# awslabs/dgl-ke

Measured on NVIDIA H100. Metric: edges/sec TransE_l2 d=400 neg=200 at 1/2/4/8 H100 vs ref CPU; HBM GB/s %peak, higher is better.
Workload: dtype f32

## Files before the change

### dgl-ke_b200/csrc/kge_abi.cu

```cuda
#include <cstdio>
#include <unistd.h>
#include <cstdarg>
#include <cstring>
#include <cstdlib>
#include <map>
#include <mutex>
#include <new>
#include <utility>
#include <cuda.h>
#include "kge_common.cuh"

namespace kge {

namespace {
thread_local char g_err[512] = "";
}

int fail(int code, const char* fmt, ...) {
  va_list ap;
  va_start(ap, fmt);
  vsnprintf(g_err, sizeof(g_err), fmt, ap);
  va_end(ap);
  return code;
}
// ... 182 lines not shown
  if (cfg->batch <= 0 || cfg->chunk_size <= 0 || cfg->neg_sample_size <= 0)
    return fail(KGE_ERR_INVALID_ARG, "batch/chunk_size/neg_sample_size must be positive");
  if (cfg->batch % cfg->chunk_size != 0)
    return fail(KGE_ERR_INVALID_ARG, "batch %lld is not a multiple of chunk_size %d", (long long)cfg->batch, cfg->chunk_size);
  const int D = cfg->entity_dim, Dr = cfg->relation_dim;
  if (D <= 0 || Dr <= 0) return fail(KGE_ERR_INVALID_ARG, "dims must be positive");
  if (D % 4 != 0 || Dr % 4 != 0)
    return fail(KGE_ERR_UNSUPPORTED, "row lengths must be multiples of 4 floats (16-byte vector/TMA access): D_e=%d D_r=%d", D, Dr);
  switch (cfg->model) {
    case KGE_TRANSE_L1: case KGE_TRANSE_L2: case KGE_DISTMULT:
      if (Dr != D) return fail(KGE_ERR_INVALID_ARG, "model needs relation_dim == entity_dim (%d vs %d)", Dr, D);
      break;
    case KGE_COMPLEX:
      if (Dr != D || D % 8 != 0) return fail(KGE_ERR_INVALID_ARG, "ComplEx needs relation_dim == entity_dim, a multiple of 8");
      break;
    case KGE_ROTATE:
      if (D != 2 * Dr || D % 8 != 0) return fail(KGE_ERR_INVALID_ARG, "RotatE needs entity_dim == 2*relation_dim (-de), a multiple of 8");
      break;
    case KGE_RESCAL:
      if (Dr != D * D) return fail(KGE_ERR_INVALID_ARG, "RESCAL needs relation_dim == entity_dim^2");
      if (D > 512) return fail(KGE_ERR_UNSUPPORTED, "RESCAL entity_dim %d > 512 is not implemented", D);
      break;
  }
  p->model = cfg->model; p->D = D; p->Dr = Dr;
  p->gamma = cfg->gamma; p->emb_init = cfg->emb_init; p->lr = cfg->lr;
  p->reg_coef = cfg->reg_coef; p->reg_norm = cfg->reg_norm;
  p->adversarial = cfg->adversarial; p->adv_temperature = cfg->adv_temperature;
  p->neg_head = cfg->neg_head ? 1 : 0;
  p->B = cfg->batch; p->Cs = cfg->chunk_size; p->Ns = cfg->neg_sample_size;
  p->C = (int)(cfg->batch / cfg->chunk_size);
  p->neg_deg = cfg->neg_deg_sample ? 1 : 0;
  if (p->neg_deg) p->Ns += p->Cs;
  p->Nn = (long long)p->C * p->Ns;
  p->U = n_nodes >= 0 ? n_nodes : 2 * p->B;
  p->U_dev = nullptr;
  p->rel_deferred = 0; p->rel_dense = 0; p->use_nc = 1; p->fused = 0; p->nc_staged = 0;
  if (cfg->loss_genre < KGE_LOSS_LOGSIGMOID || cfg->loss_genre > KGE_LOSS_BCE)
    return fail(KGE_ERR_INVALID_ARG, "loss_genre %d is not a kge_loss_t", cfg->loss_genre);
  if (cfg->pairwise && cfg->loss_genre != KGE_LOSS_HINGE && cfg->loss_genre != KGE_LOSS_LOGISTIC)
    return fail(KGE_ERR_INVALID_ARG, "pairwise needs the Hinge or the Logistic criterion (loss.py:61-62)");
  if (cfg->pairwise && cfg->adversarial)
    return fail(KGE_ERR_INVALID_ARG, "loss cannot be pairwise and adversarial sampled (base_loss.py:83-84)");
  p->hinge = cfg->loss_genre == KGE_LOSS_HINGE ? 1 : 0;
  p->margin = cfg->margin;
  p->pairwise = cfg->pairwise ? 1 : 0;
  return KGE_OK;
}

size_t align_up(size_t x, size_t a = 256) { return (x + a - 1) / a * a; }

struct CarveOpt {
  bool force_tiles = false;
  bool want_scores = true;
};

bool use_fused(kge_context* h, const StepParams& p) {
  return h->engine != 0 && h->fused_mode != 0 && fused_supported(p);
}

bool use_umma(kge_context* h, const StepParams& p) {
  return h->engine != 0 && umma_supported(p);
}

int carve(kge_context* h, const StepParams& p, StepWs* w, cudaStream_t stream, const CarveOpt& opt = CarveOpt()) {
  const size_t BD = (size_t)p.B * p.D, ND = (size_t)p.Nn * p.D, BNs = (size_t)p.B * p.Ns;
  const size_t B = (size_t)p.B, Nn = (size_t)p.Nn, U = (size_t)(p.U > 0 ? p.U : 0);
  const bool um = !opt.force_tiles && use_umma(h, p);
  const bool fused = p.fused != 0;
  const FusedHilo hl = fused ? fused_hilo(p) : FusedHilo{false, false};
  const size_t sA = B * slab_blocks(p.D) * 32 + 8192, sB = Nn * slab_blocks(p.D) * 32 + 8192;
  const size_t sV = B * slab_blocks(p.Ns) * 32 + 8192;
  const size_t sAT = (size_t)p.C * slab_blocks(p.Cs) * p.D * 32 + 8192, sBT = (size_t)p.C * slab_blocks(p.Ns) * p.D * 32 + 8192;
  const size_t sVT = (size_t)p.C * slab_blocks(p.Cs) * p.Ns * 32 + 8192;
  struct Slot { float** ptr; size_t floats; bool on; };
  const Slot slots[] = {
      {&w->NG, (U ? 2 * B : 0) * p.D, true},
      {&w->A, BD, !(um || fused)}, {&w->Bn, ND, true}, {&w->GA, BD, true}, {&w->GR, B * p.Dr, !p.rel_dense},
      {&w->S, BNs, !fused || opt.want_scores}, {&w->V, BNs, !fused},
      {&w->pos, B, true}, {&w->gpos, B, true}, {&w->pnorm, B, true}, {&w->a2, B, true}, {&w->b2, Nn, true},
      {&w->rowsum, B, true}, {&w->colsum, Nn, true}, {&w->pl, B, true}, {&w->nl, B, true}, {&w->wbar, 4, true},
      {&w->gsr, B, true}, {&w->gsn, Nn, true}, {&w->colpart, (size_t)ceil_div(p.Cs, 128) * Nn, fused},
      {&w->Mt, BD, p.model == KGE_RESCAL},
      {&w->Ahi, sA, um && (!fused || hl.a)}, {&w->Alo, sA, um && (!fused || hl.a)}, {&w->Af, sA, fused && !hl.a},
      {&w->Bhi, sB, um}, {&w->Blo, sB, um},
      {&w->Vhi, sV, um && !fused}, {&w->Vlo, sV, um && !fused},
      {&w->AhiT, sAT, um}, {&w->AloT, sAT, um}, {&w->BhiT, sBT, um}, {&w->BloT, sBT, um},
      {&w->VhiT, sVT, um && (!fused || hl.v)}, {&w->VloT, sVT, um && (!fused || hl.v)}, {&w->VT, sVT, fused},
      {&w->NC, U * p.D, p.use_nc != 0},
      {&w->regp, B + Nn + (U ? 2 * B : 0), true},
  };
  size_t need = 0;
  for (const Slot& s : slots)
    if (s.on) need += align_up(s.floats * sizeof(float));
  if (need > h->arena.bytes) {
    if (int rc = h->arena.resize(need + need / 4, stream, "step workspace")) return rc;
    h->ng_ptr = nullptr; h->ng_floats = 0;
  }
  size_t off = 0;
  for (const Slot& s : slots) {
    *s.ptr = s.on ? (float*)(h->arena.as<char>() + off) : nullptr;
    if (s.on) off += align_up(s.floats * sizeof(float));
  }
  w->red_partial = h->red_partial; w->red_ticket = (unsigned int*)(h->red_partial + 192);
  w->sync_ctr = (unsigned int*)(h->red_partial + 200);
  w->rg = nullptr; w->rgs = nullptr;
  return KGE_OK;
}

int ensure_rel_dense(kge_context* h, const TableView& rel, StepWs* w, cudaStream_t stream) {
  const size_t bytes = ((size_t)rel.num_rows * rel.dim + (size_t)rel.num_rows) * sizeof(float);
  if (bytes != h->rel_dense.bytes) {
    if (int rc = h->rel_dense.resize(bytes, stream, "relation gradient sums")) return rc;
    KGE_CUDA_OK(cudaMemsetAsync(h->rel_dense.p, 0, bytes, stream));
  }
  w->rg = h->rel_dense.as<float>();
  w->rgs = w->rg + (size_t)rel.num_rows * rel.dim;
  return KGE_OK;
}

LaunchCtx lctx(kge_context* h, void* stream) { return LaunchCtx{(cudaStream_t)stream, &h->launches, h->num_sms, &h->prof}; }

void ensure_ng_zero(kge_context* h, const StepParams& p, const StepWs& w, const LaunchCtx& c, bool force) {
  size_t n = (size_t)2 * p.B * p.D;
  if (force || h->ng_dirty || h->ng_ptr != w.NG || h->ng_floats < n) {
    launch_fill_zero(c, w.NG, (long long)n);
    h->ng_ptr = w.NG;
    h->ng_dirty = false;
  }
  h->ng_floats = n;
}

int check_batch(const kge_batch_t* b, const StepParams& p) {
  if (!b) return fail(KGE_ERR_INVALID_ARG, "batch is null");
  if (!b->node_ids || !b->head_local || !b->tail_local || !b->rel_ids || !b->neg_ids)
    return fail(KGE_ERR_INVALID_ARG, "batch has null index arrays");
  if (b->n_nodes < 0 && b->n_nodes_dev) return KGE_OK;
  if (b->n_nodes <= 0 || b->n_nodes > 2 * p.B) return fail(KGE_ERR_INVALID_ARG, "n_nodes=%lld out of (0, 2*batch]", (long long)b->n_nodes);
  return KGE_OK;
}
// ... 231 lines not shown
  if (rc) return rc;
  p.model = KGE_DISTMULT;
  DeviceGuard g(h->device);
  StepWs w{};
  rc = carve(h, p, &w, (cudaStream_t)stream);
  if (rc) return rc;
  h->ng_ptr = nullptr;
  w.V = dneg;
  w.gpos = dpos;
  launch_loss(lctx(h, stream), p, pos, neg, wt, w, log4, false);
  KGE_CUDA_OK(cudaGetLastError());
  h->have_last = false;
  return KGE_OK;
}

KGE_API int kge_adagrad(kge_handle_t h, const kge_table_t* table, const int64_t* idx, const float* grad, int64_t n, float lr,
                void* stream) {
  if (!h) return fail(KGE_ERR_INVALID_ARG, "handle is null");
  if (n < 0) return fail(KGE_ERR_INVALID_ARG, "n < 0");
  if (n == 0) return KGE_OK;
  if (!idx || !grad) return fail(KGE_ERR_INVALID_ARG, "null pointer");
  TableView v;
  int rc = make_view(table, &v, "adagrad");
  if (rc) return rc;
  DeviceGuard g(h->device);
  launch_adagrad(lctx(h, stream), v, (const long long*)idx, grad, n, lr);
  KGE_CUDA_OK(cudaGetLastError());
  return KGE_OK;
}

static int forward_backward_impl(kge_handle_t h, const kge_step_cfg_t* cfg, const kge_table_t* ent, const kge_table_t* rel,
                                 const kge_batch_t* batch, float* log4, void* stream, bool fused_step) {
  if (!h) return fail(KGE_ERR_INVALID_ARG, "handle is null");
  StepParams p;
  int rc = make_params(cfg, batch ? batch->n_nodes : 0, &p);
  if (rc) return rc;
  rc = check_batch(batch, p);
  if (rc) return rc;
  if (batch->n_nodes < 0) p.U_dev = (const long long*)batch->n_nodes_dev;
  p.rel_deferred = h->rel_deferred;
  TableView ve, vr;
  if ((rc = make_view(ent, &ve, "entity"))) return rc;
  if ((rc = make_view(rel, &vr, "relation"))) return rc;
  if (ve.dim != p.D || vr.dim != p.Dr)
    return fail(KGE_ERR_INVALID_ARG, "table dims (%d,%d) do not match cfg (%d,%d)", ve.dim, vr.dim, p.D, p.Dr);
  DeviceGuard g(h->device);
  p.fused = use_fused(h, p) ? 1 : 0;
  p.use_nc = (fused_step && ve.n_shards == 1) ? 0 : 1;
  p.rel_dense = (fused_step && p.model != KGE_RESCAL &&
                 (p.rel_deferred ? (h->ext_rg != nullptr) : ((size_t)vr.num_rows * (size_t)vr.dim <= ((size_t)64 << 20)))) ? 1 : 0;
  StepWs w{};
  CarveOpt opt;
  opt.want_scores = !fused_step;
  if ((rc = carve(h, p, &w, (cudaStream_t)stream, opt))) return rc;
  if (p.rel_dense && p.rel_deferred) { w.rg = h->ext_rg; w.rgs = h->ext_rgs; }
  else if (p.rel_dense && (rc = ensure_rel_dense(h, vr, &w, (cudaStream_t)stream))) return rc;
  LaunchCtx c = lctx(h, stream);
  BatchView b = bview(batch);
  if (p.neg_deg) {
    if (ve.n_shards != 1) return fail(KGE_ERR_UNSUPPORTED, "--neg_deg_sample needs a single-shard entity table");
    const size_t bytes = (size_t)p.Nn * sizeof(long long);
    if (bytes > h->negdeg_ids.bytes && (rc = h->negdeg_ids.resize(bytes, (cudaStream_t)stream, "neg_deg_sample id list")))
      return rc;
    launch_negdeg_ids(c, p, b, b.neg_ids, h->negdeg_ids.as<long long>());
    b.neg_ids = h->negdeg_ids.as<long long>();
  }
  ensure_ng_zero(h, p, w, c, false);
  const bool stageable = fused_step && p.fused && p.use_nc;
  float* const arena_nc = w.NC;
  h->pf.take_staged(*batch, stageable, p, w);
  const FusedPrefetch* pfp = nullptr;
  if ((rc = h->pf.arm_next(stageable, p, w, arena_nc, (cudaStream_t)stream, &pfp))) return rc;
  if (p.use_nc && !p.nc_staged) launch_gather_nodes(c, p, ve, b, w);
  if ((rc = (p.model == KGE_RESCAL) ? launch_rescal_prep(c, p, ve, vr, b, w) : launch_prep(c, p, ve, vr, b, w))) return rc;
  if (p.neg_deg) launch_negdeg_zero_reg(c, p, w);
  float* logdst = log4 ? log4 : h->dev_log4;
  if (p.fused) {
    launch_wbar(c, p, b.edge_weight, w);
    if ((rc = fused_launch(c, p, w, 0, b.edge_weight, fused_step ? nullptr : w.S, h->dump_v, &ve, b.neg_ids, pfp))) return rc;
    if ((rc = fused_launch(c, p, w, 1, b.edge_weight, nullptr,
                           h->dump_v ? h->dump_v + (size_t)p.B * p.Ns : nullptr, &ve, b.neg_ids, pfp))) return rc;
  } else {
    if ((rc = run_score(h, c, p, w))) return rc;
    if (p.neg_deg) launch_negdeg_mask_scores(c, p, w);
    launch_wbar(c, p, b.edge_weight, w);
    launch_loss_rows(c, p, w.pos, w.S, b.edge_weight, w);
    if (p.neg_deg) launch_negdeg_mask_coef(c, p, w);
    launch_colsum(c, p, w);
    if (use_umma(h, p)) {
      if ((rc = umma_grad(c, p, w, false))) return rc;
      if ((rc = umma_grad(c, p, w, true))) return rc;
    } else {
      launch_grad_a(c, p, w);
      launch_grad_b(c, p, w);
    }
    if (p.neg_deg) launch_negdeg_scatter(c, p, ve, b, w);
  }
  if (p.model == KGE_RESCAL) launch_rescal_chain(c, p, ve, vr, b, w);
  else launch_chain(c, p, ve, vr, b, w);
  if (fused_step && p.rel_deferred && !p.rel_dense && h->ext_rg) launch_rel_grad_dense(c, p, b, w, h->ext_rg, h->ext_rgs);
  if (!fused_step) launch_reduce_log(c, p, b.edge_weight, w, logdst, true);
  KGE_CUDA_OK(cudaGetLastError());
  h->last_p = p; h->last_w = w; h->last_b = b; h->last_ent = ve; h->last_rel = vr; h->have_last = true;
  h->ng_dirty = true;
  return KGE_OK;
}
// ... 432 lines not shown
```

### dgl-ke_b200/csrc/kge_common.cuh

```cuda
#pragma once
#include <cuda_runtime.h>
#include <stdint.h>
#include "../../include/kge_b200.h"

namespace kge {

constexpr int kWarp = 32;

struct TableView {
  float* emb[KGE_MAX_SHARDS];
  float* state[KGE_MAX_SHARDS];
  long long rows_per_shard;
  long long num_rows;
  int n_shards;
  int dim;
};

__device__ __forceinline__ float* row_ptr(const TableView& t, long long id) {
  if (t.n_shards == 1) return t.emb[0] + id * (long long)t.dim;
  int s = (int)(id / t.rows_per_shard);
  return t.emb[s] + (id - (long long)s * t.rows_per_shard) * (long long)t.dim;
}
__device__ __forceinline__ float* state_ptr(const TableView& t, long long id) {
  if (t.n_shards == 1) return t.state[0] + id;
// ... 324 lines not shown
void launch_adagrad(const LaunchCtx&, const TableView& t, const long long* idx, const float* grad,
                    long long n, float lr);
void launch_node_grad_with_reg(const LaunchCtx&, const StepParams&, const TableView& ent,
                               const BatchView&, const StepWs&, float* out);
void launch_fill_zero(const LaunchCtx&, float* p, long long n);
void launch_rel_grad_dense(const LaunchCtx&, const StepParams&, const BatchView&, const StepWs&, float* rg, float* rgs);
void launch_rel_apply_dense(const LaunchCtx&, const TableView& rel, float* rg, float* rgs, float lr);

void launch_negdeg_ids(const LaunchCtx&, const StepParams&, const BatchView&, const long long* sampled, long long* out);
void launch_negdeg_zero_reg(const LaunchCtx&, const StepParams&, const StepWs&);
void launch_negdeg_mask_scores(const LaunchCtx&, const StepParams&, const StepWs&);
void launch_negdeg_mask_coef(const LaunchCtx&, const StepParams&, const StepWs&);
void launch_negdeg_scatter(const LaunchCtx&, const StepParams&, const TableView& ent, const BatchView&, const StepWs&);

struct RankParams {
  const float* S;
  long long ld, Q, N;
  const float* pos;
  long long base;
  const long long* cand;
  long long chunk;
  const long long* kept;
  const long long* rel;
  const long long* keys;
  const int* vals;
  long long n_keys, n_rel;
  long long* cnt;
};
void launch_rank_count(const LaunchCtx&, const RankParams&);
void launch_rank_finish(const LaunchCtx&, const long long* cnt, long long Q, long long* rank_out, double* acc);

int launch_rescal_prep(const LaunchCtx&, const StepParams&, const TableView& ent, const TableView& rel,
                       const BatchView&, const StepWs&);
void launch_rescal_prep_dense(const LaunchCtx&, const StepParams&, const float* head, const float* relr,
                              const float* tail, const StepWs&, bool want_pos, bool want_a);
void launch_rescal_chain(const LaunchCtx&, const StepParams&, const TableView& ent, const TableView& rel,
                         const BatchView&, const StepWs&);

bool umma_supported(const StepParams&);
int umma_score(const LaunchCtx&, const StepParams&, const StepWs&);
int umma_grad(const LaunchCtx&, const StepParams&, const StepWs&, bool side_b);

struct FusedPrefetch {
  const long long* node_ids;
  const long long* nU_dev;
  long long nU;
  const long long* neg_ids;
  long long nNeg;
  float* nc;
  float* bn;
};
bool fused_supported(const StepParams&);
int fused_prefetch_slots(const StepParams& p, int mode);
struct FusedHilo { bool a, v; };
FusedHilo fused_hilo(const StepParams& p);
int fused_launch(const LaunchCtx&, const StepParams&, const StepWs&, int mode, const float* wt, float* dumpS, float* dumpV,
                 const TableView* ent, const long long* neg_ids, const FusedPrefetch* pf);

}
```

### dgl-ke_b200/csrc/kge_fused.cu

```cuda
#include <cuda.h>
#include <cstdio>
#include <cstdlib>
#include <mutex>
#include "kge_common.cuh"
#include "kge_tc.cuh"

namespace kge {

using namespace tc;

namespace {

constexpr int kTileM = 128;
constexpr int kThreadsF = 384;
constexpr int kProducerWarp = 8;
constexpr int kHandoffWarp = 9;
constexpr int kMaxS1 = 4, kMaxS2 = 8;
constexpr int kMaxPf = 8;
constexpr uint32_t kRingBytes = 192 * 1024;
constexpr uint32_t kRingBytesP = 223 * 1024;
constexpr float kLog2e = 1.4426950408889634f;
constexpr float kLn2 = 0.6931471805599453f;

struct FusedArgs {
  int model, adversarial;
  float gamma, Tl2e, inv2B, uni;
  float reg_coef;
  int reg_norm;
  int C, Rx, Ry, D;
  int N1;
  int N2;
  int nblkD;
  int nS1, nS2;
  uint32_t stage1Bytes, stage2Bytes;
  float* VT;
  float *VhiT, *VloT;
  float* colpart;
  int ncolpart;
  const float* x2;
  const float* y2;
  const float* pos;
  const float* wt;
  const float* wbar;
  float *gpos, *rowsum, *pl, *nl;
  float* dumpS;
  float* dumpV;
  const float *Xhi, *Xlo;
  const long long* xids;
  TableView xtab;
  const float* xraw;
  float* gsn;
  float* out;
  int pf_slots;
  int pf_parity;
  int pf_lag;
  uint32_t pf_off, pf_row_bytes;
  const long long* pf_node_ids;
  const long long* pf_nU_dev;
  long long pf_nU, pf_nNeg;
  const long long* pf_neg_ids;
  float* pf_nc;
  float* pf_bn;
};

static __device__ __noinline__ float reg_grad_any(float b, int norm, float coef) { return reg_grad(b, norm, coef); }
__device__ __forceinline__ float reg_grad_fast(float b, int norm, float coef) {
  if (norm == 3) return 3.f * coef * fabsf(b) * b;
  return reg_grad_any(b, norm, coef);
}

__device__ __forceinline__ void epi_bar() { asm volatile("bar.sync 1, 256;" ::: "memory"); }

__device__ __forceinline__ void prefetch_rows(const FusedArgs& g, uint8_t* ring, uint64_t (*pf_full)[kMaxPf], int w, int lane) {
  const int S = g.pf_slots;
  const long long nU = g.pf_nU_dev ? *g.pf_nU_dev : g.pf_nU;
  const long long total = nU + g.pf_nNeg;
  const long long nhalf = total > g.pf_parity ? (total - g.pf_parity + 1) / 2 : 0;
  const long long stride = 2ll * gridDim.x, j0 = 2ll * blockIdx.x + w;
  const long long n = j0 < nhalf ? (nhalf - j0 + stride - 1) / stride : 0;
  uint8_t* slots = ring + g.pf_off + (size_t)w * S * g.pf_row_bytes;
  auto vrow = [&](long long k) { return g.pf_parity + 2 * (j0 + k * stride); };
  auto fetch_ids = [&](long long kb) {
    const long long k = kb + lane;
    if (k >= n) return 0ll;
    const long long v = vrow(k);
    return v < nU ? g.pf_node_ids[v] : g.pf_neg_ids[v - nU];
  };
// ... 401 lines not shown
        float acc2[NW / 2];
#pragma unroll
        for (int i = 0; i < NW / 2; ++i) acc2[i] = 0.f;
        uint32_t ah[2][4], al[2][4];
#pragma unroll 1
        for (int kb = 0; kb < nkb2; ++kb) {
          const uint32_t s = n2 % g.nS2;
          mbar_wait(&full2[s], (n2 / g.nS2) & 1);
          const uint32_t st = smem_u32(ring2 + (size_t)s * g.stage2Bytes);
          const uint64_t dYh = make_desc(st), dYl = make_desc(st + yBytes2);
          const int kleft = g.Ry - kb * 32;
          const int ksteps = kleft >= 32 ? 4 : (kleft >> 3);
#pragma unroll
          for (int ks = 0; ks < 4; ++ks) {
            const int j = kb * 4 + ks;
            if (ks < ksteps) {
              const uint64_t o = (uint64_t)(ks * 2);
              pos_kstep<NW>(acc2, ah[j & 1], al[j & 1], vw + j * 128, dYh + o, dYl + o);
              if (j > 0) {
                wgmma_wait<1>();
                reg_fence(ah[(j - 1) & 1]); reg_fence(al[(j - 1) & 1]);
                if (ks == 0 && lane == 0) mbar_arrive(&empty2[(n2 - 1) % g.nS2]);
              }
            }
          }
          ++n2;
        }
        wgmma_wait<0>();
        reg_fence(ah[0]); reg_fence(ah[1]); reg_fence(al[0]); reg_fence(al[1]);
        if (lane == 0) mbar_arrive(&empty2[(n2 - 1) % g.nS2]);
        reg_fence(acc2);
#pragma unroll
        for (int h = 0; h < 2; ++h) {
          const int m = m0 + rloc + 8 * h;
          if (m >= g.Rx) continue;
          float* orow = g.out + ((long long)c * g.Rx + m) * (long long)g.D;
#pragma unroll
          for (int j = 0; j < NW / 8; ++j) {
            const int k = d0 + 8 * j + 2 * q;
            if (k >= g.D) continue;
            *reinterpret_cast<float2*>(orow + k) = make_float2(acc2[4 * j + 2 * h] * rscal[h], acc2[4 * j + 2 * h + 1] * rscal[h]);
          }
        }
      }
      asm volatile("fence.proxy.async.shared::cta;" ::: "memory");
      __syncwarp();
      if (lane == 0) mbar_arrive(&vfree);
    }
  }
}

constexpr int kNegEpiLoads = 16;

template <int NW, bool FLAT>
__global__ void __launch_bounds__(kThreadsF, 1)
k_fused_neg(const __grid_constant__ CUtensorMap mV, const __grid_constant__ CUtensorMap mVl,
            const __grid_constant__ CUtensorMap mAh, const __grid_constant__ CUtensorMap mAl, FusedArgs g) {
  extern __shared__ __align__(1024) uint8_t smem_raw[];
  __shared__ __align__(8) uint64_t full[kMaxS1], empty[kMaxS1];
  __shared__ __align__(8) uint64_t pf_full[2][kMaxPf];

  const int warp = threadIdx.x >> 5, lane = threadIdx.x & 31;
  uint8_t* ring = (uint8_t*)(((uintptr_t)smem_raw + 1023) & ~(uintptr_t)1023);

  const int mtiles = (g.Rx + kTileM - 1) / kTileM;
  const int ntiles = g.C * mtiles;
  const int nkb = (g.Ry + 31) >> 5;
  const int nch = (g.D + NW - 1) / NW;
  constexpr uint32_t aBytes = (uint32_t)kTileM * 128u;
  constexpr uint32_t bBytes = (uint32_t)NW * 128u;
  constexpr uint32_t vBytes = k_reg_a(NW) ? aBytes : 2u * aBytes;
  const bool l2 = g.model == KGE_TRANSE_L2;

  if (threadIdx.x == 0) {
    for (int s = 0; s < kMaxS1; ++s) { mbar_init(&full[s], 1); mbar_init(&empty[s], 8); }
    for (int s = 0; s < kMaxPf; ++s) { mbar_init(&pf_full[0][s], 1); mbar_init(&pf_full[1][s], 1); }
    asm volatile("fence.mbarrier_init.release.cluster;" ::: "memory");
  }
  if (warp == kProducerWarp && lane == 0) {
    tma_prefetch_desc(&mV); if (!k_reg_a(NW)) tma_prefetch_desc(&mVl); tma_prefetch_desc(&mAh); tma_prefetch_desc(&mAl);
  }
  __syncthreads();

  if (warp >= 8) {
  asm volatile("setmaxnreg.dec.sync.aligned.u32 56;");
  if (warp == kProducerWarp) {
    uint32_t n = 0;
    for (int tile = blockIdx.x; tile < ntiles; tile += gridDim.x) {
      const int c = tile / mtiles, m0 = (tile % mtiles) * kTileM;
      for (int ch = 0; ch < nch; ++ch) {
        for (int kb = 0; kb < nkb; ++kb, ++n) {
          const uint32_t s = n % g.nS1;
          mbar_wait(&empty[s], ((n / g.nS1) & 1) ^ 1);
          uint8_t* st = ring + (size_t)s * g.stage1Bytes;
          const int yv = (c * nkb + kb) * g.Rx + m0;
          const int ya = (c * nkb + kb) * g.D + ch * NW;
          if (elect_one()) {
            mbar_expect_tx(&full[s], vBytes + 2u * bBytes);
            tma_load_2d(st, &mV, &full[s], 0, yv);
            if (!k_reg_a(NW)) tma_load_2d(st + aBytes, &mVl, &full[s], 0, yv);
            tma_load_2d(st + vBytes, &mAh, &full[s], 0, ya);
            tma_load_2d(st + vBytes + bBytes, &mAl, &full[s], 0, ya);
          }
          __syncwarp();
        }
      }
    }
  } else if (warp >= 10 && g.pf_slots > 0) {
    prefetch_rows(g, ring, pf_full, warp - 10, lane);
  }
  } else {
    asm volatile("setmaxnreg.inc.sync.aligned.u32 224;");
    const int wg = warp >> 2, q = lane & 3;
    const int et = threadIdx.x;
    const int rloc = wg * 64 + (warp & 3) * 16 + (lane >> 2);
    uint32_t n = 0;
    for (int tile = blockIdx.x; tile < ntiles; tile += gridDim.x) {
      const int c = tile / mtiles, m0 = (tile % mtiles) * kTileM;
      if (g.dumpV) {
        for (int e = et; e < kTileM * g.Ry; e += 256) {
          const int j = m0 + e / g.Ry, i = e % g.Ry;
          if (j >= g.Rx) break;
          const long long o = slabT_off(c, g.Ry, g.Rx, i, j);
          float hi, lo;
          if (k_reg_a(NW)) split_tf32(g.VT[o], hi, lo);
          else { hi = g.VhiT[o]; lo = g.VloT[o]; }
          g.dumpV[((long long)c * g.Rx + j) * g.Ry + i] = hi + lo;
        }
      }
      float cs[2] = {0.f, 0.f};
      if (l2) {
#pragma unroll
        for (int h = 0; h < 2; ++h) {
          const int m = m0 + rloc + 8 * h;
          if (m >= g.Rx) continue;
          const float* p = g.colpart + (long long)c * g.Rx + m;
          for (int t = 0; t < g.ncolpart; ++t) cs[h] += p[(long long)t * g.C * g.Rx];
        }
      }
// ... 74 lines not shown
              wgmma_wait<1>();
              if (lane == 0) mbar_arrive(&empty[(n - 1) % g.nS1]);
            }
          }
          if (early) load_b(0, d0, 0);
          wgmma_wait<0>();
        }
        if (lane == 0) mbar_arrive(&empty[(n - 1) % g.nS1]);
        reg_fence(acc);
#pragma unroll
        for (int h = 0; h < 2; ++h) {
          if (!rok[h]) continue;
          float* orow = g.out + ((long long)c * g.Rx + m0 + rloc + 8 * h) * (long long)g.D;
#pragma unroll
          for (int j0 = 0; j0 < NJ; j0 += NB) {
            if (!early || h > 0 || j0 > 0) load_b(h, d0, j0);
#pragma unroll
            for (int jj = 0; jj < NB; ++jj) {
              const int j = j0 + jj;
              const int k = d0 + 8 * j + 2 * q;
              if (j >= NJ || k >= g.D) continue;
              float o0 = acc[4 * j + 2 * h], o1 = acc[4 * j + 2 * h + 1];
              const float2 b = FLAT ? bh[jj] : make_float2(bh[jj].x + bl[jj].x, bh[jj].y + bl[jj].y);
              if (l2) { o0 = fmaf(b.x, -cs[h], o0); o1 = fmaf(b.y, -cs[h], o1); }
              o0 += reg_grad_fast(b.x, g.reg_norm, g.reg_coef);
              o1 += reg_grad_fast(b.y, g.reg_norm, g.reg_coef);
              gsq[h] += o0 * o0 + o1 * o1;
              *reinterpret_cast<float2*>(orow + k) = make_float2(o0, o1);
            }
          }
        }
      }
#pragma unroll
      for (int h = 0; h < 2; ++h) {
        float v = gsq[h];
        v += __shfl_xor_sync(0xffffffffu, v, 1);
        v += __shfl_xor_sync(0xffffffffu, v, 2);
        const int m = m0 + rloc + 8 * h;
        if (q == 0 && m < g.Rx) g.gsn[(long long)c * g.Rx + m] = v / (float)g.D;
      }
    }
  }
}

}

bool fused_supported(const StepParams& p) {
  return umma_supported(p) && !p.hinge && !p.pairwise && !p.neg_deg && p.Cs <= 240 && p.Ns <= 240;
}

namespace {
constexpr uint32_t kLoBytes = (uint32_t)kTileM * 128u;
uint32_t stage1_bytes(int n) { return (k_reg_a(n) ? 1u : 2u) * kLoBytes + 2u * (uint32_t)n * 128u; }
struct Geometry { int Rx, Ry, N1, N2, nS1, nS2, pf_slots; uint32_t ringBytes, stage1Bytes, stage2Bytes, pf_off; bool ok; };

int neg_chunk_width(int D, bool want_prefetch) {
  static const int widths[] = {64, 128, 200, 256};
  int best = 0;
  long long best_rows = 0;
  for (int w : widths) {
    if (w == 256 && want_prefetch) continue;
    const long long rows = (long long)((D + w - 1) / w) * (kTileM + w);
    if (!best || rows < best_rows) { best = w; best_rows = rows; }
  }
  return best;
}

Geometry geometry(const StepParams& p, int mode, bool want_prefetch) {
  Geometry q{};
  const uint32_t row = (uint32_t)p.D * 4u;
  if (mode == 1) {
    q.Rx = p.Ns; q.Ry = p.Cs;
    q.ringBytes = kRingBytes;
    q.N1 = neg_chunk_width(p.D, want_prefetch);
    q.stage1Bytes = stage1_bytes(q.N1);
    q.nS1 = (int)(kRingBytes / q.stage1Bytes); if (q.nS1 > kMaxS1) q.nS1 = kMaxS1;
    q.ok = q.nS1 >= 2;
    if (q.ok && want_prefetch) {
      const uint32_t fp = stage1_bytes(q.N1) + (k_reg_a(q.N1) ? kLoBytes : 0u);
      int nS = (int)(kRingBytes / fp); if (nS > kMaxS1) nS = kMaxS1;
      while (nS > 2 && kRingBytes - (uint32_t)nS * fp < 2u * kMaxPf * row) --nS;
      const uint32_t used = (uint32_t)nS * fp;
      int slots = (int)((kRingBytes - used) / (2u * row));
      if (slots > kMaxPf) slots = kMaxPf;
      if (slots >= 2 && nS >= 2) { q.pf_slots = slots; q.nS1 = nS; q.pf_off = used; }
    }
    return q;
  }
  q.Rx = p.Cs; q.Ry = p.Ns;
  q.N1 = q.Ry <= 64 ? 64 : (q.Ry <= 128 ? 128 : (q.Ry <= 208 ? 208 : 256));
  const uint32_t ring = want_prefetch ? kRingBytes : kRingBytesP;
  q.ringBytes = ring;
  q.stage1Bytes = stage1_bytes(q.N1);
  const uint32_t fp1 = (want_prefetch && k_reg_a(q.N1)) ? q.stage1Bytes + kLoBytes : q.stage1Bytes;
  int nS1 = (int)(ring / fp1); if (nS1 > kMaxS1) nS1 = kMaxS1;
  if (nS1 < 2) return q;
  const uint32_t vBytes = (uint32_t)q.N1 * 512u;
  const bool w200 = (p.D + 199) / 200 * 200 < (p.D + 127) / 128 * 128;
  const int widths[2] = {w200 ? 200 : 128, w200 ? 128 : 200};
  Geometry first{};
  for (int NW : widths) {
    Geometry t = q;
    t.N2 = NW;
    t.stage2Bytes = 2u * (uint32_t)NW * 128u;
    if (vBytes + 2u * t.stage2Bytes > ring) continue;
    t.nS1 = nS1;
    t.nS2 = (int)((ring - vBytes) / t.stage2Bytes); if (t.nS2 > kMaxS2) t.nS2 = kMaxS2;
    t.ok = true;
    if (!want_prefetch) return t;
    if (!first.ok) first = t;
    const uint32_t want = 2u * kMaxPf * row;
    int s1 = t.nS1, s2 = t.nS2;
    while (s1 > 2 && ring - (uint32_t)s1 * fp1 < want) --s1;
    while (s2 > 2 && ring - (vBytes + (uint32_t)s2 * t.stage2Bytes) < want) --s2;
    uint32_t used = (uint32_t)s1 * fp1;
    if (vBytes + (uint32_t)s2 * t.stage2Bytes > used) used = vBytes + (uint32_t)s2 * t.stage2Bytes;
    int slots = (int)((ring - used) / (2u * row));
    if (slots > kMaxPf) slots = kMaxPf;
    if (slots >= 2) { t.pf_slots = slots; t.nS1 = s1; t.nS2 = s2; t.pf_off = used; return t; }
  }
  return first;
}

int launch_error() {
  const cudaError_t e = cudaGetLastError();
  return e == cudaSuccess ? KGE_OK : fail(KGE_ERR_CUDA, "k_fused launch: %s", cudaGetErrorString(e));
}
const char* pos_launch_name(int NV, int NW, int pf) {
  static const int nvs[4] = {64, 128, 208, 256}, nws[2] = {128, 200};
  static char names[4][2][kMaxPf + 1][96];
  static std::once_flag once;
  std::call_once(once, [] {
    for (int a = 0; a < 4; ++a)
      for (int b = 0; b < 2; ++b)
        for (int f = 0; f <= kMaxPf; ++f)
          snprintf(names[a][b][f], sizeof(names[a][b][f]), "k_fused<P: S=A.Bn^T, loss, GA=V.Bn> NV=%d NW=%d pf=%d hand=%d",
                   nvs[a], nws[b], f, f > 0 ? 1 : 3);
  });
  const int a = NV == 64 ? 0 : NV == 128 ? 1 : NV == 208 ? 2 : 3;
  return names[a][NW == 200][pf < 0 ? 0 : (pf > kMaxPf ? kMaxPf : pf)];
}
template <int NV, int NW>
int launch_pos(const LaunchCtx& c, int grid, size_t smem, const CUtensorMap* m, const FusedArgs& g) {
  if (int rc = smem_optin((const void*)k_fused_pos<NV, NW>, smem)) return rc;
  KGE_LAUNCH_NAMED(c, pos_launch_name(NV, NW, g.pf_slots), (k_fused_pos<NV, NW>), grid, kThreadsF, smem,
                   m[0], m[1], m[2], m[3], m[4], m[5], g);
  return launch_error();
}
template <int NV>
int launch_pos(const LaunchCtx& c, int grid, size_t smem, const CUtensorMap* m, const FusedArgs& g) {
  if constexpr (NV < 256) {
    if (g.N2 == 200) return launch_pos<NV, 200>(c, grid, smem, m, g);
  }
  return launch_pos<NV, 128>(c, grid, smem, m, g);
}
template <int NW, bool FLAT>
int launch_neg_src(const LaunchCtx& c, int grid, size_t smem, const CUtensorMap* m, const FusedArgs& g) {
  if (int rc = smem_optin((const void*)k_fused_neg<NW, FLAT>, smem)) return rc;
  static char name[64];
  static std::once_flag once;
  std::call_once(once, [] { snprintf(name, sizeof(name), "k_fused<N: G_neg=V^T.A, mean sq> NW=%d", NW); });
  KGE_LAUNCH_NAMED(c, name, (k_fused_neg<NW, FLAT>), grid, kThreadsF, smem, m[0], m[1], m[2], m[3], g);
  return launch_error();
}
template <int NW>
int launch_neg(const LaunchCtx& c, int grid, size_t smem, const CUtensorMap* m, const FusedArgs& g) {
  return (g.xraw || g.xids) ? launch_neg_src<NW, true>(c, grid, smem, m, g) : launch_neg_src<NW, false>(c, grid, smem, m, g);
}
int launch_width(const LaunchCtx& c, bool P, int grid, size_t smem, const CUtensorMap* m, const FusedArgs& g) {
  switch (g.N1) {
    case 64: return P ? launch_pos<64>(c, grid, smem, m, g) : launch_neg<64>(c, grid, smem, m, g);
    case 128: return P ? launch_pos<128>(c, grid, smem, m, g) : launch_neg<128>(c, grid, smem, m, g);
    case 200: return launch_neg<200>(c, grid, smem, m, g);
    case 208: return launch_pos<208>(c, grid, smem, m, g);
    default: return P ? launch_pos<256>(c, grid, smem, m, g) : launch_neg<256>(c, grid, smem, m, g);
  }
}
}

int fused_prefetch_slots(const StepParams& p, int mode) { return geometry(p, mode, true).pf_slots; }

FusedHilo fused_hilo(const StepParams& p) {
  return FusedHilo{!k_reg_a(geometry(p, 0, false).N1), !k_reg_a(neg_chunk_width(p.D, false))};
}

int fused_launch(const LaunchCtx& c, const StepParams& p, const StepWs& w, int mode, const float* wt, float* dumpS,
                 float* dumpV, const TableView* ent, const long long* neg_ids, const FusedPrefetch* pf) {
  FusedArgs g{};
  g.model = p.model; g.adversarial = p.adversarial;
  g.gamma = p.gamma; g.Tl2e = p.adv_temperature * kLog2e; g.inv2B = 0.5f / (float)p.B; g.uni = 1.f / (float)p.Ns;
  g.reg_coef = p.reg_coef; g.reg_norm = p.reg_norm;
  g.C = p.C; g.D = p.D; g.nblkD = slab_blocks(p.D);
  const bool P = mode == 0;
  const Geometry q = geometry(p, mode, pf != nullptr && ent != nullptr);
  if (!q.ok) return fail(KGE_ERR_UNSUPPORTED, "fused kernel: shape does not fit (N1=%d)", q.N1);
  g.Rx = q.Rx; g.Ry = q.Ry; g.N1 = q.N1; g.N2 = q.N2; g.nS1 = q.nS1; g.nS2 = q.nS2;
  g.stage1Bytes = q.stage1Bytes; g.stage2Bytes = q.stage2Bytes;
  if (pf && ent && q.pf_slots >= 2) {
    static const int lag_env = getenv("KGE_B200_PF_LAG") ? atoi(getenv("KGE_B200_PF_LAG")) : 1;
    g.pf_lag = lag_env < 1 ? 1 : (lag_env > 3 ? 3 : lag_env);
    g.pf_slots = q.pf_slots; g.pf_off = q.pf_off; g.pf_row_bytes = (uint32_t)p.D * 4u; g.pf_parity = mode;
    g.pf_node_ids = pf->node_ids; g.pf_nU_dev = pf->nU_dev; g.pf_nU = pf->nU; g.pf_nNeg = pf->nNeg;
    g.pf_neg_ids = pf->neg_ids; g.pf_nc = pf->nc; g.pf_bn = pf->bn;
    g.xtab = *ent;
  }
  if (k_reg_a(geometry(p, 1, pf != nullptr && ent != nullptr).N1)) g.VT = w.VT;
  else { g.VhiT = w.VhiT; g.VloT = w.VloT; }
  g.colpart = w.colpart; g.ncolpart = (p.Cs + kTileM - 1) / kTileM;
  g.dumpV = dumpV;
  const size_t smem = q.ringBytes + 1024;
  const int mtiles = (g.Rx + kTileM - 1) / kTileM;
  int grid = p.C * mtiles;
  if (grid > c.num_sms) grid = c.num_sms;
  CUtensorMap m[6];
  if (P) {
    g.x2 = w.a2; g.y2 = w.b2;
    g.pos = w.pos; g.wt = wt; g.wbar = w.wbar;
    g.gpos = w.gpos; g.rowsum = w.rowsum; g.pl = w.pl; g.nl = w.nl;
    g.dumpS = dumpS;
    g.out = w.GA;
    const long long rowsX = (long long)p.C * p.Cs * g.nblkD, rowsY = (long long)p.C * p.Ns * g.nblkD;
    const long long rowsYT = (long long)p.C * slab_blocks(p.Ns) * p.D;
    const bool ra = k_reg_a(g.N1);
    if (tc_make_map(&m[0], ra ? w.Af : w.Ahi, rowsX, 32, kTileM) || tc_make_map(&m[1], ra ? w.Af : w.Alo, rowsX, 32, kTileM) ||
        tc_make_map(&m[2], w.Bhi, rowsY, 32, g.N1) || tc_make_map(&m[3], w.Blo, rowsY, 32, g.N1) ||
        tc_make_map(&m[4], w.BhiT, rowsYT, 32, g.N2) || tc_make_map(&m[5], w.BloT, rowsYT, 32, g.N2))
      return KGE_ERR_CUDA;
    return launch_width(c, true, grid, smem, m, g);
  }
  g.Xhi = w.Bhi; g.Xlo = w.Blo;
  if (ent && ent->n_shards == 1 && neg_ids) { g.xids = neg_ids; g.xtab = *ent; }
  if (w.BnRaw) g.xraw = w.BnRaw;
  g.gsn = w.gsn;
  g.out = w.Bn;
  const long long rowsV = (long long)p.C * slab_blocks(p.Cs) * p.Ns, rowsA = (long long)p.C * slab_blocks(p.Cs) * p.D;
  const bool rv = k_reg_a(g.N1);
  if (tc_make_map(&m[0], rv ? w.VT : w.VhiT, rowsV, 32, kTileM) || tc_make_map(&m[1], rv ? w.VT : w.VloT, rowsV, 32, kTileM) ||
      tc_make_map(&m[2], w.AhiT, rowsA, 32, g.N1) || tc_make_map(&m[3], w.AloT, rowsA, 32, g.N1))
    return KGE_ERR_CUDA;
  return launch_width(c, false, grid, smem, m, g);
}

}
```

Before: 35.57 million.

## Build transposed A hi/lo TF32 slabs on-chip in fused negative-gradient kernel

Adds an on-chip path for the fused negative-side kernel. Four converter warps TMA-load the flat A tiles into a landing buffer in shared memory, transpose them, split them into TF32 hi/lo parts and write them into the MMA stage ring. This removes the precomputed A^T hi/lo slabs from global memory, along with their workspace and HBM traffic. In exchange it adds shared-memory conversion work, a second mbarrier ring and fewer pipeline stages, and it is only enabled when prefetch is off and the shape fits.

```diff
diff --git a/dgl-ke_b200/csrc/kge_abi.cu b/dgl-ke_b200/csrc/kge_abi.cu
--- a/dgl-ke_b200/csrc/kge_abi.cu
+++ b/dgl-ke_b200/csrc/kge_abi.cu
@@ -258,6 +258,7 @@
 struct CarveOpt {
   bool force_tiles = false;
   bool want_scores = true;
+  bool may_prefetch = false;
 };
 
 bool use_fused(kge_context* h, const StepParams& p) {
@@ -273,7 +274,7 @@
   const size_t B = (size_t)p.B, Nn = (size_t)p.Nn, U = (size_t)(p.U > 0 ? p.U : 0);
   const bool um = !opt.force_tiles && use_umma(h, p);
   const bool fused = p.fused != 0;
-  const FusedHilo hl = fused ? fused_hilo(p) : FusedHilo{false, false};
+  const FusedHilo hl = fused ? fused_hilo(p, opt.may_prefetch) : FusedHilo{false, false, false};
   const size_t sA = B * slab_blocks(p.D) * 32 + 8192, sB = Nn * slab_blocks(p.D) * 32 + 8192;
   const size_t sV = B * slab_blocks(p.Ns) * 32 + 8192;
   const size_t sAT = (size_t)p.C * slab_blocks(p.Cs) * p.D * 32 + 8192, sBT = (size_t)p.C * slab_blocks(p.Ns) * p.D * 32 + 8192;
@@ -290,7 +291,7 @@
       {&w->Ahi, sA, um && (!fused || hl.a)}, {&w->Alo, sA, um && (!fused || hl.a)}, {&w->Af, sA, fused && !hl.a},
       {&w->Bhi, sB, um}, {&w->Blo, sB, um},
       {&w->Vhi, sV, um && !fused}, {&w->Vlo, sV, um && !fused},
-      {&w->AhiT, sAT, um}, {&w->AloT, sAT, um}, {&w->BhiT, sBT, um}, {&w->BloT, sBT, um},
+      {&w->AhiT, sAT, um && !hl.aT_chip}, {&w->AloT, sAT, um && !hl.aT_chip}, {&w->BhiT, sBT, um}, {&w->BloT, sBT, um},
       {&w->VhiT, sVT, um && (!fused || hl.v)}, {&w->VloT, sVT, um && (!fused || hl.v)}, {&w->VT, sVT, fused},
       {&w->NC, U * p.D, p.use_nc != 0},
       {&w->regp, B + Nn + (U ? 2 * B : 0), true},
@@ -628,6 +629,7 @@
   StepWs w{};
   CarveOpt opt;
   opt.want_scores = !fused_step;
+  opt.may_prefetch = fused_step && p.use_nc;
   if ((rc = carve(h, p, &w, (cudaStream_t)stream, opt))) return rc;
   if (p.rel_dense && p.rel_deferred) { w.rg = h->ext_rg; w.rgs = h->ext_rgs; }
   else if (p.rel_dense && (rc = ensure_rel_dense(h, vr, &w, (cudaStream_t)stream))) return rc;
diff --git a/dgl-ke_b200/csrc/kge_common.cuh b/dgl-ke_b200/csrc/kge_common.cuh
--- a/dgl-ke_b200/csrc/kge_common.cuh
+++ b/dgl-ke_b200/csrc/kge_common.cuh
@@ -400,8 +400,8 @@
 };
 bool fused_supported(const StepParams&);
 int fused_prefetch_slots(const StepParams& p, int mode);
-struct FusedHilo { bool a, v; };
-FusedHilo fused_hilo(const StepParams& p);
+struct FusedHilo { bool a, v, aT_chip; };
+FusedHilo fused_hilo(const StepParams& p, bool may_prefetch);
 int fused_launch(const LaunchCtx&, const StepParams&, const StepWs&, int mode, const float* wt, float* dumpS, float* dumpV,
                  const TableView* ent, const long long* neg_ids, const FusedPrefetch* pf);
 
diff --git a/dgl-ke_b200/csrc/kge_fused.cu b/dgl-ke_b200/csrc/kge_fused.cu
--- a/dgl-ke_b200/csrc/kge_fused.cu
+++ b/dgl-ke_b200/csrc/kge_fused.cu
@@ -1,6 +1,7 @@
 #include <cuda.h>
 #include <cstdio>
 #include <cstdlib>
+#include <cstring>
 #include <mutex>
 #include "kge_common.cuh"
 #include "kge_tc.cuh"
@@ -17,6 +18,9 @@
 constexpr int kHandoffWarp = 9;
 constexpr int kMaxS1 = 4, kMaxS2 = 8;
 constexpr int kMaxPf = 8;
+constexpr int kConvWarp = 8, kConvWarps = 4;
+constexpr int kMaxL = 2;
+constexpr uint32_t kBoxBytes = 32u * 128u;
 constexpr uint32_t kRingBytes = 192 * 1024;
 constexpr uint32_t kRingBytesP = 223 * 1024;
 constexpr float kLog2e = 1.4426950408889634f;
@@ -33,6 +37,9 @@
   int nblkD;
   int nS1, nS2;
   uint32_t stage1Bytes, stage2Bytes;
+  int aT_chip;
+  int nL;
+  uint32_t land_off, land_bytes;
   float* VT;
   float *VhiT, *VloT;
   float* colpart;
@@ -540,12 +547,109 @@
 
 constexpr int kNegEpiLoads = 16;
 
+__device__ __forceinline__ void sts_f32x4(uint32_t a, float x, float y, float z, float w) {
+  asm volatile("st.shared.v4.f32 [%0], {%1, %2, %3, %4};" ::"r"(a), "f"(x), "f"(y), "f"(z), "f"(w) : "memory");
+}
+
+template <int NW>
+__device__ __forceinline__ void build_at(const FusedArgs& g, uint8_t* ring, const CUtensorMap* mV, const CUtensorMap* mAf,
+                                         uint64_t* lfull, uint64_t* lempty, uint64_t* full, uint64_t* empty, int cw,
+                                         int lane) {
+  constexpr uint32_t aBytes = (uint32_t)kTileM * 128u;
+  constexpr uint32_t bBytes = (uint32_t)NW * 128u;
+  constexpr int ncg = (NW + 31) / 32;
+  const int mtiles = (g.Rx + kTileM - 1) / kTileM;
+  const int ntiles = g.C * mtiles;
+  const int nkb = (g.Ry + 31) >> 5;
+  const int nch = (g.D + NW - 1) / NW;
+  const uint32_t ring_s = smem_u32(ring);
+  const uint32_t per_tile = (uint32_t)(nch * nkb);
+  const uint32_t total = blockIdx.x < (uint32_t)ntiles ? ((ntiles - 1 - blockIdx.x) / gridDim.x + 1) * per_tile : 0u;
+  auto land_load = [&](uint32_t m) {
+    const int tile = blockIdx.x + (int)(m / per_tile) * gridDim.x, r = (int)(m % per_tile);
+    const int c = tile / mtiles, ch = r / nkb, kb = r % nkb;
+    const int d0 = ch * NW, db0 = d0 >> 5;
+    const int nbox = ((d0 & 31) + (g.D - d0 < NW ? g.D - d0 : NW) + 31) >> 5;
+    const uint32_t l = m % g.nL;
+    if (elect_one()) {
+      mbar_expect_tx(&lfull[l], (uint32_t)nbox * kBoxBytes);
+      for (int b = 0; b < nbox; ++b)
+        tma_load_2d(ring + g.land_off + (size_t)l * g.land_bytes + (size_t)b * kBoxBytes, mAf, &lfull[l], 0,
+                    (c * g.nblkD + db0 + b) * g.Ry + kb * 32);
+    }
+    __syncwarp();
+  };
+  if (cw == 0)
+    for (uint32_t m = 0; m < (uint32_t)g.nL && m < total; ++m) land_load(m);
+  uint32_t n = 0;
+  for (int tile = blockIdx.x; tile < ntiles; tile += gridDim.x) {
+    const int c = tile / mtiles, m0 = (tile % mtiles) * kTileM;
+    for (int ch = 0; ch < nch; ++ch) {
+      const int d0 = ch * NW, off = d0 & 31;
+      const int ncols = g.D - d0 < NW ? g.D - d0 : NW;
+      for (int kb = 0; kb < nkb; ++kb, ++n) {
+        const uint32_t l = n % g.nL, s = n % g.nS1;
+        mbar_wait(&empty[s], ((n / g.nS1) & 1) ^ 1);
+        if (cw == 0) {
+          if (elect_one()) {
+            mbar_expect_tx(&full[s], aBytes);
+            tma_load_2d(ring + (size_t)s * g.stage1Bytes, mV, &full[s], 0, (c * nkb + kb) * g.Rx + m0);
+          }
+          __syncwarp();
+        }
+        mbar_wait(&lfull[l], (n / g.nL) & 1);
+        const uint32_t land = ring_s + g.land_off + l * g.land_bytes;
+        const uint32_t hi = ring_s + s * g.stage1Bytes + aBytes, lo = hi + bBytes;
+        const int kleft = g.Ry - kb * 32;
+        const int nks = kleft >= 32 ? 4 : (kleft >> 3);
+        int cg = 0, ks = cw;
+        while (ks >= nks) { ks -= nks; ++cg; }
+        for (; cg < ncg;) {
+          const int d = 32 * cg + lane;
+          if (d < NW) {
+            float v[8];
+            if (d < ncols) {
+              const int e = off + d;
+              const uint32_t src = land + (uint32_t)(e >> 5) * kBoxBytes + (uint32_t)(8 * ks) * 128u + (uint32_t)((e & 3) << 2);
+              const int ec = (e >> 2) & 7;
+#pragma unroll
+              for (int t = 0; t < 8; ++t) v[t] = lds_f32(src + (uint32_t)t * 128u + (uint32_t)((ec ^ t) << 4));
+            } else {
+#pragma unroll
+              for (int t = 0; t < 8; ++t) v[t] = 0.f;
+            }
+            float h[8], o[8];
+#pragma unroll
+            for (int t = 0; t < 8; ++t) split_tf32(v[t], h[t], o[t]);
+#pragma unroll
+            for (int c2 = 0; c2 < 2; ++c2) {
+              const uint32_t dst = (uint32_t)d * 128u + (uint32_t)((((2 * ks + c2) ^ (d & 7))) << 4);
+              sts_f32x4(hi + dst, h[4 * c2], h[4 * c2 + 1], h[4 * c2 + 2], h[4 * c2 + 3]);
+              sts_f32x4(lo + dst, o[4 * c2], o[4 * c2 + 1], o[4 * c2 + 2], o[4 * c2 + 3]);
+            }
+          }
+          ks += kConvWarps;
+          while (ks >= nks) { ks -= nks; ++cg; }
+        }
+        asm volatile("fence.proxy.async.shared::cta;" ::: "memory");
+        __syncwarp();
+        if (lane == 0) { mbar_arrive(&lempty[l]); mbar_arrive(&full[s]); }
+        if (cw == 0 && n + g.nL < total) {
+          mbar_wait(&lempty[l], (n / g.nL) & 1);
+          land_load(n + g.nL);
+        }
+      }
+    }
+  }
+}
+
 template <int NW, bool FLAT>
 __global__ void __launch_bounds__(kThreadsF, 1)
 k_fused_neg(const __grid_constant__ CUtensorMap mV, const __grid_constant__ CUtensorMap mVl,
             const __grid_constant__ CUtensorMap mAh, const __grid_constant__ CUtensorMap mAl, FusedArgs g) {
   extern __shared__ __align__(1024) uint8_t smem_raw[];
   __shared__ __align__(8) uint64_t full[kMaxS1], empty[kMaxS1];
+  __shared__ __align__(8) uint64_t lfull[kMaxL], lempty[kMaxL];
   __shared__ __align__(8) uint64_t pf_full[2][kMaxPf];
 
   const int warp = threadIdx.x >> 5, lane = threadIdx.x & 31;
@@ -559,20 +663,25 @@
   constexpr uint32_t bBytes = (uint32_t)NW * 128u;
   constexpr uint32_t vBytes = k_reg_a(NW) ? aBytes : 2u * aBytes;
   const bool l2 = g.model == KGE_TRANSE_L2;
+  const bool chip = k_reg_a(NW) && g.aT_chip;
 
   if (threadIdx.x == 0) {
-    for (int s = 0; s < kMaxS1; ++s) { mbar_init(&full[s], 1); mbar_init(&empty[s], 8); }
+    for (int s = 0; s < kMaxS1; ++s) { mbar_init(&full[s], chip ? 1 + kConvWarps : 1); mbar_init(&empty[s], 8); }
+    for (int s = 0; s < kMaxL; ++s) { mbar_init(&lfull[s], 1); mbar_init(&lempty[s], kConvWarps); }
     for (int s = 0; s < kMaxPf; ++s) { mbar_init(&pf_full[0][s], 1); mbar_init(&pf_full[1][s], 1); }
     asm volatile("fence.mbarrier_init.release.cluster;" ::: "memory");
   }
   if (warp == kProducerWarp && lane == 0) {
-    tma_prefetch_desc(&mV); if (!k_reg_a(NW)) tma_prefetch_desc(&mVl); tma_prefetch_desc(&mAh); tma_prefetch_desc(&mAl);
+    tma_prefetch_desc(&mV); if (!k_reg_a(NW)) tma_prefetch_desc(&mVl); tma_prefetch_desc(&mAh);
+    if (!chip) tma_prefetch_desc(&mAl);
   }
   __syncthreads();
 
   if (warp >= 8) {
   asm volatile("setmaxnreg.dec.sync.aligned.u32 56;");
-  if (warp == kProducerWarp) {
+  if (chip) {
+    if constexpr (k_reg_a(NW)) build_at<NW>(g, ring, &mV, &mAh, lfull, lempty, full, empty, warp - kConvWarp, lane);
+  } else if (warp == kProducerWarp) {
     uint32_t n = 0;
     for (int tile = blockIdx.x; tile < ntiles; tile += gridDim.x) {
       const int c = tile / mtiles, m0 = (tile % mtiles) * kTileM;
@@ -753,7 +862,11 @@
 namespace {
 constexpr uint32_t kLoBytes = (uint32_t)kTileM * 128u;
 uint32_t stage1_bytes(int n) { return (k_reg_a(n) ? 1u : 2u) * kLoBytes + 2u * (uint32_t)n * 128u; }
-struct Geometry { int Rx, Ry, N1, N2, nS1, nS2, pf_slots; uint32_t ringBytes, stage1Bytes, stage2Bytes, pf_off; bool ok; };
+struct Geometry {
+  int Rx, Ry, N1, N2, nS1, nS2, pf_slots, nL;
+  uint32_t ringBytes, stage1Bytes, stage2Bytes, pf_off, land_off, land_bytes;
+  bool ok;
+};
 
 int neg_chunk_width(int D, bool want_prefetch) {
   static const int widths[] = {64, 128, 200, 256};
@@ -767,7 +880,16 @@
   return best;
 }
 
-Geometry geometry(const StepParams& p, int mode, bool want_prefetch) {
+uint32_t landing_bytes(int D, int NW) {
+  int most = 0;
+  for (int d0 = 0; d0 < D; d0 += NW) {
+    const int nbox = ((d0 & 31) + (D - d0 < NW ? D - d0 : NW) + 31) >> 5;
+    if (nbox > most) most = nbox;
+  }
+  return (uint32_t)most * kBoxBytes;
+}
+
+Geometry geometry(const StepParams& p, int mode, bool want_prefetch, bool chip = false) {
   Geometry q{};
   const uint32_t row = (uint32_t)p.D * 4u;
   if (mode == 1) {
@@ -775,6 +897,17 @@
     q.ringBytes = kRingBytes;
     q.N1 = neg_chunk_width(p.D, want_prefetch);
     q.stage1Bytes = stage1_bytes(q.N1);
+    if (chip && k_reg_a(q.N1) && !want_prefetch) {
+      q.land_bytes = landing_bytes(p.D, q.N1);
+      const uint32_t land = kMaxL * q.land_bytes;
+      q.nS1 = land < kRingBytes ? (int)((kRingBytes - land) / q.stage1Bytes) : 0;
+      if (q.nS1 > kMaxS1) q.nS1 = kMaxS1;
+      q.land_off = (uint32_t)q.nS1 * q.stage1Bytes;
+      q.nL = (int)((kRingBytes - q.land_off) / q.land_bytes);
+      if (q.nL > kMaxL) q.nL = kMaxL;
+      q.ok = q.nL >= 1 && q.nS1 >= 2;
+      return q;
+    }
     q.nS1 = (int)(kRingBytes / q.stage1Bytes); if (q.nS1 > kMaxS1) q.nS1 = kMaxS1;
     q.ok = q.nS1 >= 2;
     if (q.ok && want_prefetch) {
@@ -858,10 +991,13 @@
 template <int NW, bool FLAT>
 int launch_neg_src(const LaunchCtx& c, int grid, size_t smem, const CUtensorMap* m, const FusedArgs& g) {
   if (int rc = smem_optin((const void*)k_fused_neg<NW, FLAT>, smem)) return rc;
-  static char name[64];
+  static char name[2][80];
   static std::once_flag once;
-  std::call_once(once, [] { snprintf(name, sizeof(name), "k_fused<N: G_neg=V^T.A, mean sq> NW=%d", NW); });
-  KGE_LAUNCH_NAMED(c, name, (k_fused_neg<NW, FLAT>), grid, kThreadsF, smem, m[0], m[1], m[2], m[3], g);
+  std::call_once(once, [] {
+    for (int chip = 0; chip < 2; ++chip)
+      snprintf(name[chip], sizeof(name[chip]), "k_fused<N: G_neg=V^T.A, mean sq> aT=%s NW=%d", chip ? "chip" : "slab", NW);
+  });
+  KGE_LAUNCH_NAMED(c, name[g.aT_chip ? 1 : 0], (k_fused_neg<NW, FLAT>), grid, kThreadsF, smem, m[0], m[1], m[2], m[3], g);
   return launch_error();
 }
 template <int NW>
@@ -881,8 +1017,12 @@
 
 int fused_prefetch_slots(const StepParams& p, int mode) { return geometry(p, mode, true).pf_slots; }
 
-FusedHilo fused_hilo(const StepParams& p) {
-  return FusedHilo{!k_reg_a(geometry(p, 0, false).N1), !k_reg_a(neg_chunk_width(p.D, false))};
+FusedHilo fused_hilo(const StepParams& p, bool may_prefetch) {
+  FusedHilo f{!k_reg_a(geometry(p, 0, false).N1), !k_reg_a(neg_chunk_width(p.D, false)), false};
+  const char* slab_env = getenv("KGE_B200_FUSED_SLAB_T");
+  const bool forced = slab_env && slab_env[0] && strcmp(slab_env, "0") != 0;
+  f.aT_chip = !may_prefetch && !forced && !f.a && !f.v && p.model != KGE_RESCAL && geometry(p, 1, false, true).ok;
+  return f;
 }
 
 int fused_launch(const LaunchCtx& c, const StepParams& p, const StepWs& w, int mode, const float* wt, float* dumpS,
@@ -893,10 +1033,15 @@
   g.reg_coef = p.reg_coef; g.reg_norm = p.reg_norm;
   g.C = p.C; g.D = p.D; g.nblkD = slab_blocks(p.D);
   const bool P = mode == 0;
-  const Geometry q = geometry(p, mode, pf != nullptr && ent != nullptr);
+  const bool want_prefetch = pf != nullptr && ent != nullptr;
+  const bool chip = !P && w.AhiT == nullptr;
+  if (chip && want_prefetch) return fail(KGE_ERR_UNSUPPORTED, "fused kernel: prefetch slots need the A^T slabs");
+  const Geometry q = geometry(p, mode, want_prefetch, chip);
   if (!q.ok) return fail(KGE_ERR_UNSUPPORTED, "fused kernel: shape does not fit (N1=%d)", q.N1);
+  if (chip && (q.nL < 1 || !w.Af)) return fail(KGE_ERR_UNSUPPORTED, "fused kernel: no A^T slabs and no on-chip form (N1=%d)", q.N1);
   g.Rx = q.Rx; g.Ry = q.Ry; g.N1 = q.N1; g.N2 = q.N2; g.nS1 = q.nS1; g.nS2 = q.nS2;
   g.stage1Bytes = q.stage1Bytes; g.stage2Bytes = q.stage2Bytes;
+  g.aT_chip = chip ? 1 : 0; g.nL = q.nL; g.land_off = q.land_off; g.land_bytes = q.land_bytes;
   if (pf && ent && q.pf_slots >= 2) {
     static const int lag_env = getenv("KGE_B200_PF_LAG") ? atoi(getenv("KGE_B200_PF_LAG")) : 1;
     g.pf_lag = lag_env < 1 ? 1 : (lag_env > 3 ? 3 : lag_env);
@@ -935,10 +1080,16 @@
   g.gsn = w.gsn;
   g.out = w.Bn;
   const long long rowsV = (long long)p.C * slab_blocks(p.Cs) * p.Ns, rowsA = (long long)p.C * slab_blocks(p.Cs) * p.D;
+  const long long rowsAf = (long long)p.C * g.nblkD * p.Cs;
   const bool rv = k_reg_a(g.N1);
-  if (tc_make_map(&m[0], rv ? w.VT : w.VhiT, rowsV, 32, kTileM) || tc_make_map(&m[1], rv ? w.VT : w.VloT, rowsV, 32, kTileM) ||
-      tc_make_map(&m[2], w.AhiT, rowsA, 32, g.N1) || tc_make_map(&m[3], w.AloT, rowsA, 32, g.N1))
+  if (tc_make_map(&m[0], rv ? w.VT : w.VhiT, rowsV, 32, kTileM) || tc_make_map(&m[1], rv ? w.VT : w.VloT, rowsV, 32, kTileM))
     return KGE_ERR_CUDA;
+  if (chip) {
+    if (tc_make_map(&m[2], w.Af, rowsAf, 32, 32)) return KGE_ERR_CUDA;
+    m[3] = m[2];
+  } else if (tc_make_map(&m[2], w.AhiT, rowsA, 32, g.N1) || tc_make_map(&m[3], w.AloT, rowsA, 32, g.N1)) {
+    return KGE_ERR_CUDA;
+  }
   return launch_width(c, false, grid, smem, m, g);
 }
 
```

New measurement: 36.47 million (median of 6 runs). +2.5%, better.
